# microsoft/esvit

Hardware: NVIDIA H100
Metric: multi-crop images/sec, Swin-T W7 pretrain step (2 global 224^2 + 8 local 96^2 crops, DDINOLoss V+R, K=65536) (higher is better)
Workload: dtype bf16

## Files before the change

esvit_b200/_lib.py:

```python
from __future__ import annotations

import ctypes
import os
from ctypes import c_double, c_float, c_int, c_longlong, c_void_p

HERE = os.path.dirname(os.path.abspath(__file__))
LIB_PATH = os.path.join(HERE, "lib", "libesvit_b200.so")
HEADER_PATH = os.path.join(os.path.dirname(HERE), "include", "esvit_b200.h")

ERR_BAD_ARG = 1001

P, I, L, F, D = c_void_p, c_int, c_longlong, c_float, c_double

SIGNATURES = {
    "esvit_add_ln_fwd": [P, P, P, I, P, P, F, P, P, I, P, P, L, I, P],
    "esvit_add_ln_bwd": [P, I, P, P, P, P, P, P, I, P, P, P, P, P, L, I, P],
    "esvit_patch_merge_ln_fwd": [P, P, P, F, P, P, P, I, I, I, I, P],
    "esvit_patch_merge_ln_bwd": [P, P, P, P, P, P, P, P, I, I, I, I, P],
    "esvit_token_mean_fwd": [P, P, I, I, I, P],
    "esvit_token_mean_bwd": [P, P, P, I, I, I, P],
    "esvit_patch_embed_fwd": [P, P, P, P, P, F, P, P, P, I, I, I, I, P],
    "esvit_patch_embed_bwd": [P, P, P, P, P, P, P, P, P, P, P, I, I, I, I, P],
    "esvit_window_attn_expand_bias": [P, P, I, I, P],
    "esvit_window_attn_fwd": [P, P, P, P, I, P, P, I, I, I, I, I, I, I, F, P],
    "esvit_window_attn_bwd": [P, P, P, P, I, P, P, P, P, P, P, I, I, I, I, I, I, I, F, P],
    "esvit_window_attn_probs": [P, P, P, P, I, P, I, I, I, I, I, I, I, F, P],
    "esvit_gemm_bias_act": [P, P, P, P, P, L, I, I, I, P],
    "esvit_gemm_mul_colsum": [P, P, P, P, P, P, L, I, I, P],
    "esvit_gemm_bf16": [P, P, P, P, P, L, I, I, I, I, I, I, P],
    "esvit_gemm_mul_colsum2": [P, P, P, P, P, P, L, I, I, I, I, P],
    "esvit_gemm_wgrad_ws_floats": [I, I],
    "esvit_gemm_wgrad": [P, P, P, P, L, I, I, I, I, P],
    "esvit_mlp_fwd": [P, P, P, P, P, P, P, P, L, I, P],
    "esvit_gelu_fwd": [P, P, L, P],
    "esvit_gelu_bwd": [P, P, P, L, P],
    "esvit_gelu_bwd_dbias": [P, P, P, P, L, I, P],
    "esvit_mul_bwd_dbias": [P, P, P, P, L, I, P],
    "esvit_l2norm_fwd": [P, P, P, F, L, I, P],
    "esvit_l2norm_bwd": [P, P, P, P, L, I, P],
    "esvit_weight_norm_fwd": [P, P, P, P, L, I, P],
    "esvit_weight_norm_bwd": [P, P, P, P, I, P, P, L, I, P],
    "esvit_row_lse": [P, P, F, P, L, I, P],
    "esvit_dino_ce_fwd": [P, P, P, P, P, P, P, F, F, P, L, I, P],
    "esvit_dino_ce_bwd": [P, P, P, P, P, P, P, P, P, F, F, P, L, I, P],
    "esvit_weighted_sum": [P, P, I, P, P],
    "esvit_row_softmax_q_max_k": [],
    "esvit_row_softmax_q": [P, P, F, P, P, L, I, P],
    "esvit_dino_ce_q_fwd": [P, P, P, P, P, F, P, L, I, P],
    "esvit_dino_ce_q_bwd": [P, P, P, P, P, P, P, F, P, L, I, P],
    "esvit_mixup_q_kpad": [I],
    "esvit_mixup_q": [P, P, I, I, I, F, P, P, P, P],
    "esvit_colsum_workspace_rows": [],
    "esvit_colsum": [P, L, I, P, P, P],
    "esvit_center_ema": [P, P, F, F, P, I, P],
    "esvit_normalize_rows": [P, P, L, I, F, P],
    "esvit_region_match": [P, P, I, I, I, I, I, P, P, P],
# ... 75 lines not shown
    if rc != 0:
        if rc == ERR_BAD_ARG:
            raise ValueError(f"{name}: unsupported shape / argument (ESVIT_ERR_BAD_ARG)")
        raise EsvitKernelError(f"{name} failed: {_cuda_error_string(rc)} (status {rc})")


_LAUNCHES = {"esvit_colsum": 2, "esvit_gemm_mul_colsum": 2, "esvit_gemm_mul_colsum2": 2, "esvit_gemm_wgrad": 2,
             "esvit_mixup_q": 2}
_launch_count = 0
_timed_names = set()
_timed_events = []
_META = {
    "esvit_dino_ce_bwd": lambda a: {"rows": int(a[-3]), "K": int(a[-2])},
    "esvit_window_attn_bwd": lambda a: _attn_meta(a),
    "esvit_window_attn_fwd": lambda a: _attn_meta(a),
    "esvit_window_attn_probs": lambda a: _attn_meta(a),
    "esvit_gemm_bias_act": lambda a: {"M": int(a[5]), "N": int(a[6]), "K": int(a[7])},
    "esvit_gemm_mul_colsum": lambda a: {"M": int(a[6]), "N": int(a[7]), "K": int(a[8])},
    "esvit_gemm_bf16": lambda a: {"M": int(a[5]), "N": int(a[6]), "K": int(a[7]), "b_mn": int(a[9]), "act": int(a[10]),
                                  "pre": a[4] is not None and a[4].value is not None},
    "esvit_gemm_mul_colsum2": lambda a: {"M": int(a[6]), "N": int(a[7]), "K": int(a[8])},
    "esvit_gemm_wgrad": lambda a: {"T": int(a[4]), "N": int(a[5]), "K": int(a[6])},
    "esvit_mlp_fwd": lambda a: {"M": int(a[8]), "C": int(a[9]), "student": a[6] is not None and a[6].value is not None},
    "esvit_add_ln_fwd": lambda a: {"T": int(a[-3]), "C": int(a[-2]), "has_x": a[0] is not None and a[0].value is not None,
                                   "has_delta": a[1] is not None and a[1].value is not None},
    "esvit_add_ln_bwd": lambda a: {"T": int(a[-3]), "C": int(a[-2])},
    "esvit_dino_ce_fwd": lambda a: {"rows": int(a[-3]), "K": int(a[-2])},
    "esvit_dino_ce_q_fwd": lambda a: {"rows": int(a[-3]), "K": int(a[-2])},
    "esvit_dino_ce_q_bwd": lambda a: {"rows": int(a[-3]), "K": int(a[-2])},
    "esvit_row_softmax_q": lambda a: {"rows": int(a[-3]), "K": int(a[-2])},
    "esvit_mixup_q": lambda a: {"ncrops": int(a[2]), "B": int(a[3]), "K": int(a[4])},
    "esvit_conv_im2col": lambda a: {"B": int(a[3]), "C": int(a[4]), "H": int(a[5]), "W": int(a[6]), "k": int(a[7]),
                                    "s": int(a[8]), "p": int(a[9]), "Kp": int(a[10])},
    "esvit_conv_col2im": lambda a: {"B": int(a[2]), "C": int(a[3]), "H": int(a[4]), "W": int(a[5]), "k": int(a[6]),
                                    "s": int(a[7]), "p": int(a[8]), "Kp": int(a[9])},
    "esvit_dwbn_fwd_stats": lambda a: {"B": int(a[5]), "H": int(a[6]), "W": int(a[7]), "Hp": int(a[8]), "Wp": int(a[9]),
                                       "C": int(a[10])},
    "esvit_dwbn_fwd_apply": lambda a: {"N": int(a[9]), "C": int(a[10])},
    "esvit_dwbn_bwd_stats": lambda a: {"N": int(a[7]), "C": int(a[8])},
    "esvit_dwbn_bwd_apply": lambda a: {"B": int(a[10]), "H": int(a[11]), "W": int(a[12]), "Hp": int(a[13]),
                                       "Wp": int(a[14]), "C": int(a[15])},
    "esvit_mhsa_win_fwd": lambda a: {"B": int(a[3]), "H": int(a[4]), "W": int(a[5]), "w": int(a[6]), "C": int(a[7]),
                                     "nH": int(a[8])},
    "esvit_mhsa_win_bwd": lambda a: {"B": int(a[6]), "H": int(a[7]), "W": int(a[8]), "w": int(a[9]), "C": int(a[10]),
                                     "nH": int(a[11])},
    "esvit_vil_sc_fwd": lambda a: {"B": int(a[8]), "nx": int(a[9]), "ny": int(a[10]), "nH": int(a[11])},
# ... 70 lines not shown
```

esvit_b200/backbone.py:

```python
from __future__ import annotations

from typing import Dict, List, Optional, Sequence

import torch
import torch.nn as nn

from . import ops, shadow

Tensor = torch.Tensor


class _CastCache:

    def __init__(self):
        self.d: Dict[int, Tensor] = {}

    def __call__(self, p: Optional[Tensor]) -> Optional[Tensor]:
        if p is None:
            return None
        k = id(p)
        t = self.d.get(k)
        if t is None:
            t = self.d[k] = shadow.as_bf16(p)
        return t
# ... 37 lines not shown
    r = torch.rand(kp.shape[0], samples, dtype=torch.float32, device=device)
    return r.add_(kp).floor_().div_(kp)


def row_samples(owner: nn.Module, counts, device) -> Tensor:
    counts = tuple(counts)

    def make():
        rows = torch.tensor([L for B, L in counts for _ in range(B)])
        return torch.arange(rows.numel()).repeat_interleave(rows).to(device)
    return _cached(owner, ("rows", counts, device), make)


def drop_path_rows(owner: nn.Module, scales: Optional[Tensor], counts, device) -> Optional[Tensor]:
    return None if scales is None else scales.index_select(1, row_samples(owner, counts, device))


def block_keeps(block: nn.Module, B: int, L: int, device) -> List[Optional[Tensor]]:
    ks = [drop_path_scales(block, [block.drop_prob], B, device) for _ in range(2)]
    return [None if k is None else drop_path_rows(block, k, ((B, L),), device)[0] for k in ks]


def pre_norm_block(x: Optional[Tensor], pend, norm1: nn.Module, attend, norm2: nn.Module, attn_bias: Optional[Tensor],
                   mlp, mlp_bias: Optional[Tensor], k1: Optional[Tensor], k2: Optional[Tensor]):
    delta, keep, dbias = pend if pend is not None else (None, None, None)
    x, y = ops.add_layer_norm(x, delta, keep, norm1.weight, norm1.bias, norm1.eps, delta_bias=dbias)
    x, y = ops.add_layer_norm(x, attend(y), k1, norm2.weight, norm2.bias, norm2.eps, delta_bias=attn_bias)
    return x, (mlp(y), k2, mlp_bias)


def tap(taps, b: int, x: Tensor, pend, geometry):
    if taps is None or taps[b] is None:
        return x, pend
    x = ops.residual_add(x, *pend)
    taps[b](x, geometry)
    return x, None


def check_crops(imgs: Sequence[Tensor]) -> None:
    for im in imgs:
        if im.dim() != 4 or im.shape[1] != 3:
            raise ValueError(f"expected crops [B, 3, H, W], got {tuple(im.shape)}")


class MultiCropBackbone(nn.Module):

    def _final_norm(self, x: Tensor, pend) -> Tensor:
        delta, keep, dbias = pend if pend is not None else (None, None, None)
        _, y = ops.add_layer_norm(x, delta, keep, self.norm.weight, self.norm.bias, self.norm.eps, y_bf16=False,
                                  delta_bias=dbias)
# ... 42 lines not shown
```

esvit_b200/csrc/gemm2_wgmma.cu:

```cuda
#include <cuda.h>

#include "common.cuh"

namespace hg {

constexpr int BK = 64;
constexpr int FOLD_THREADS = 64;
constexpr int SMEM_LIMIT = 232448;
enum { EPI_BIAS = 0, EPI_GELU = 1, EPI_MUL = 2, EPI_F32 = 3 };

__device__ __forceinline__ uint32_t smem_u32(const void* p) { return (uint32_t)__cvta_generic_to_shared(p); }
__device__ __forceinline__ void mbar_init(uint64_t* bar, uint32_t count) {
  asm volatile("mbarrier.init.shared::cta.b64 [%0], %1;\n" ::"r"(smem_u32(bar)), "r"(count));
}
__device__ __forceinline__ void mbar_expect_tx(uint64_t* bar, uint32_t bytes) {
  asm volatile("mbarrier.arrive.expect_tx.shared::cta.b64 _, [%0], %1;\n" ::"r"(smem_u32(bar)), "r"(bytes) : "memory");
}
__device__ __forceinline__ void mbar_arrive(uint64_t* bar) {
  asm volatile("mbarrier.arrive.shared::cta.b64 _, [%0];\n" ::"r"(smem_u32(bar)) : "memory");
}
__device__ __forceinline__ uint64_t global_ns() {
  uint64_t t;
  asm volatile("mov.u64 %0, %%globaltimer;\n" : "=l"(t));
  return t;
}
__device__ __forceinline__ void mbar_wait(uint64_t* bar, uint32_t parity) {
  const uint32_t a = smem_u32(bar);
  uint32_t done = 0;
  uint64_t t0 = 0;
  for (uint32_t it = 0;; ++it) {
    asm volatile(
        "{\n\t.reg .pred p;\n\t"
// ... 134 lines not shown
__device__ __forceinline__ float gelu_fwd(float x) {
  const float x2 = x * x;
  const float th = tanh_approx(x * fmaf(GELU_B, x2, GELU_A));
  const float hx = 0.5f * x;
  return fmaf(hx, th, hx);
}
__device__ __forceinline__ float gelu_fwd_grad(float x, float& dy) {
  const float x2 = x * x;
  const float th = tanh_approx(x * fmaf(GELU_B, x2, GELU_A));
  const float hx = 0.5f * x;
  const float m = fmaf(th, th, -1.f);
  const float nc = fmaf(-3.f * GELU_B, x2, -GELU_A);
  dy = fmaf(hx * m, nc, fmaf(0.5f, th, 0.5f));
  return fmaf(hx, th, hx);
}
constexpr float QGELU_A = 1.702f;
__device__ __forceinline__ float qgelu_fwd(float x) { return x * __frcp_rn(1.f + __expf(-QGELU_A * x)); }
__device__ __forceinline__ float qgelu_fwd_grad(float x, float& dy) {
  const float s = __frcp_rn(1.f + __expf(-QGELU_A * x));
  dy = s * fmaf(QGELU_A * x, 1.f - s, 1.f);
  return x * s;
}

struct Params {
  const float* bias;
  bf16* out;
  bf16* aux;
  float* colsum;
  float* part;
  int M, N, K;
  int splits;
  int kb_per_split;
};

template <int WG, int BN, int EPI>
struct Cfg {
  static constexpr bool PP = WG == 1;
  static constexpr int NEP = PP ? 2 : 1;
  static constexpr int BM = 64 * WG;
  static constexpr int A_BYTES = BM * BK * 2;
  static constexpr int B_BYTES = BN * BK * 2;
  static constexpr int STAGE_BYTES = A_BYTES + B_BYTES;
  static constexpr int BAR_BYTES = PP ? 512 : 256;
  static constexpr int NCHUNK = BN / 64;
  static constexpr int CHUNK_BYTES = BM * 128;
  static constexpr int EP_WG_BYTES = EPI == EPI_BIAS ? 2 * CHUNK_BYTES
                                   : EPI == EPI_GELU ? 4 * CHUNK_BYTES
                                   : EPI == EPI_MUL  ? NCHUNK * CHUNK_BYTES : 0;
  static constexpr int EP_BYTES = NEP * EP_WG_BYTES;
  static constexpr int CS_BYTES = EPI == EPI_MUL ? 8 * BN * 4 : 0;
  static constexpr int STAGES_RAW = (SMEM_LIMIT - 1024  - BAR_BYTES - EP_BYTES - CS_BYTES) / STAGE_BYTES;
  static constexpr int STAGES = STAGES_RAW > 6 ? 6 : STAGES_RAW;
  static constexpr int SMEM = 1024 + STAGES * STAGE_BYTES + EP_BYTES + CS_BYTES + BAR_BYTES;
  static constexpr int NTHREADS = 384;
  static_assert(STAGES >= (BN == 256 && (WG == 2 || EPI == EPI_MUL) ? 3 : 4), "operand ring too shallow");
  static_assert(SMEM <= SMEM_LIMIT, "shared memory budget");
  static_assert((2 * STAGES + 2 * NEP + 2 * NEP * NCHUNK + 2) * 8 <= BAR_BYTES, "mbarrier area");
};

template <int WG, int BN, int EPI, int AMN, int BMN, bool QUICK = false>
__global__ void __launch_bounds__(384, 1) gemm_kernel(const __grid_constant__ CUtensorMap map_a,
                                                      const __grid_constant__ CUtensorMap map_b,
                                                      const __grid_constant__ CUtensorMap map_o,
                                                      const __grid_constant__ CUtensorMap map_x,
                                                      const Params p) {
  using C = Cfg<WG, BN, EPI>;
  constexpr int STAGES = C::STAGES, BM = C::BM, NCHUNK = C::NCHUNK;
  constexpr bool PP = C::PP;
  extern __shared__ __align__(1024) uint8_t smem_raw[];
// ... 94 lines not shown
    const int frag_row = row0 + warp * 16 + (lane >> 2);
    const int frag_col = 2 * (lane & 3);
    const uint32_t rows_off = PP ? 0u : (uint32_t)wg * 8192u;
    const int e = PP ? wg : 0;
    uint8_t* const my_ep = ep + e * C::EP_WG_BYTES;
    constexpr uint32_t KSTEP_A = AMN ? (2048 >> 4) : (32 >> 4), KSTEP_B = BMN ? (2048 >> 4) : (32 >> 4);
    int stage = 0;
    uint32_t phase = 0;
    int local = 0;
    for (int item = blockIdx.x; item < num_items; item += gridDim.x, local++) {
      const int tile = item % tiles_mn, split = item / tiles_mn;
      const int m0 = (tile / n_tiles) * BM, n0 = (tile % n_tiles) * BN;
      const int kb0 = split * p.kb_per_split;
      int kb1 = kb0 + p.kb_per_split; kb1 = kb1 < k_blocks ? kb1 : k_blocks;
      if constexpr (PP) {
        if ((local & 1) != wg) {
          stage += kb1 - kb0;
          while (stage >= STAGES) { stage -= STAGES; phase ^= 1; }
          continue;
        }
        if (local > 0) mbar_wait(&turn[wg], ((local - 1) >> 1) & 1);
      }
      const int use = PP ? local >> 1 : local;
      float acc[BN / 2];
      int prev = -1;
      for (int kb = kb0; kb < kb1; kb++) {
        mbar_wait(&full[stage], phase);
        const uint32_t sa = smem_u32(tiles + stage * C::STAGE_BYTES) + rows_off;
        const uint64_t da = make_smem_desc(sa, AMN), db = make_smem_desc(smem_u32(tiles + stage * C::STAGE_BYTES) + C::A_BYTES, BMN);
        wgmma_fence();
#pragma unroll
        for (int k = 0; k < BK / 16; k++)
          wgmma_tile<BN, AMN, BMN>(acc, da + k * KSTEP_A, db + k * KSTEP_B, (kb > kb0 || k != 0) ? 1u : 0u);
        wgmma_commit();
        wgmma_wait<1>();
        if (prev >= 0) mbar_arrive(&empty[prev]);
        prev = stage;
        if (++stage == STAGES) { stage = 0; phase ^= 1; }
      }
      if constexpr (PP) mbar_arrive(&turn[wg ^ 1]);
      wgmma_wait<0>();
      if (prev >= 0) mbar_arrive(&empty[prev]);

      if constexpr (EPI == EPI_F32) {
#pragma unroll
        for (int i = 0; i < BN / 8; i++) {
          const int col = n0 + i * 8 + frag_col;
          if (col >= p.N) continue;
#pragma unroll
          for (int h = 0; h < 2; h++) {
            const int row = m0 + frag_row + 8 * h;
            if (row >= p.M) continue;
            const long long off = (long long)row * p.N + col;
            *reinterpret_cast<float2*>(p.part + (long long)split * p.M * p.N + off) =
                make_float2(acc[4 * i + 2 * h], acc[4 * i + 2 * h + 1]);
          }
        }
        continue;
      }

      if constexpr (EPI == EPI_MUL) mbar_wait(&cs_empty[e], (use & 1) ^ 1);
      const uint32_t lrow = (uint32_t)(warp * 16 + (lane & 15)) * 128u, lsw = lane & 7, lblk = lane >> 4;
      const bool leader = t == 0;
#pragma unroll
      for (int c = 0; c < NCHUNK; c++) {
        uint32_t buf;
        if constexpr (EPI == EPI_MUL) {
          buf = smem_u32(my_ep + c * C::CHUNK_BYTES) + rows_off;
          mbar_wait(&mul_full[e * NCHUNK + c], use & 1);
        } else {
          buf = smem_u32(my_ep + (c & 1) * (EPI == EPI_GELU ? 2 : 1) * C::CHUNK_BYTES) + rows_off;
        }
#pragma unroll
        for (int jj = 0; jj < 8; jj += 2) {
          const int i = c * 8 + jj;
          const uint32_t addr = buf + lrow + (((jj + lblk) ^ lsw) << 4);
          const float* a0 = acc + 4 * i;
          if constexpr (EPI == EPI_MUL) {
            uint32_t m[4];
            ldmatrix_x4(addr, m[0], m[1], m[2], m[3]);
            uint32_t o[4];
            float cs[2][2] = {{0.f, 0.f}, {0.f, 0.f}};
#pragma unroll
            for (int q = 0; q < 4; q++) {
              const float2 mf = unpack_bf162(m[q]);
              o[q] = pack_bf162(a0[2 * q] * mf.x, a0[2 * q + 1] * mf.y);
              const float2 of = unpack_bf162(o[q]);
              cs[q >> 1][0] += of.x; cs[q >> 1][1] += of.y;
            }
            stmatrix_x4(addr, o[0], o[1], o[2], o[3]);
#pragma unroll
            for (int s = 0; s < 2; s++) {
              float cs0 = cs[s][0], cs1 = cs[s][1];
#pragma unroll
              for (int o2 = 4; o2 < 32; o2 <<= 1) {
                cs0 += __shfl_xor_sync(0xffffffffu, cs0, o2);
                cs1 += __shfl_xor_sync(0xffffffffu, cs1, o2);
              }
              if (lane < 4)
                *reinterpret_cast<float2*>(cs_part + (wg * 4 + warp) * BN + (i + s) * 8 + frag_col) = make_float2(cs0, cs1);
            }
          } else {
            float b[4] = {0.f, 0.f, 0.f, 0.f};
            if (p.bias) {
#pragma unroll
              for (int s = 0; s < 2; s++) {
                const int col = n0 + (i + s) * 8 + frag_col;
                if (col < p.N) {
                  const float2 bb = __ldg(reinterpret_cast<const float2*>(p.bias + col));
                  b[2 * s] = bb.x; b[2 * s + 1] = bb.y;
                }
              }
            }
            uint32_t o[4], d[4];
#pragma unroll
            for (int q = 0; q < 4; q++) {
              const float v0 = a0[2 * q] + b[2 * (q >> 1)], v1 = a0[2 * q + 1] + b[2 * (q >> 1) + 1];
              if constexpr (EPI == EPI_GELU) {
                if (p.aux) {
                  float d0, d1;
                  float y0, y1;
                  if constexpr (QUICK) {
                    y0 = qgelu_fwd_grad(v0, d0); y1 = qgelu_fwd_grad(v1, d1);
                  } else {
// ... 385 lines not shown
    if (!c.a_mn) return c.b_mn ? launch_cfg<WG, BN, EPI, 0, 1>(c, stream, rows_out) : launch_cfg<WG, BN, EPI, 0, 0>(c, stream, rows_out);
    return c.b_mn ? launch_cfg<WG, BN, EPI, 1, 1>(c, stream, rows_out) : launch_cfg<WG, BN, EPI, 1, 0>(c, stream, rows_out);
  }
  return ESVIT_ERR_BAD_ARG;
}

template <int EPI>
static int launch_epi(const Call& c, int wg, int bn, void* stream, int* rows_out) {
  if (wg == 2 && bn == 256) return launch_majors<2, 256, EPI>(c, stream, rows_out);
  if (wg == 2 && bn == 128) return launch_majors<2, 128, EPI>(c, stream, rows_out);
  if (wg == 1 && bn == 256) return launch_majors<1, 256, EPI>(c, stream, rows_out);
  if (wg == 1 && bn == 128) return launch_majors<1, 128, EPI>(c, stream, rows_out);
  return ESVIT_ERR_BAD_ARG;
}

static int launch_quick(const Call& c, int wg, int bn, void* stream) {
  if (c.a_mn || c.b_mn) return ESVIT_ERR_BAD_ARG;
  if (wg == 2 && bn == 256) return launch_cfg<2, 256, EPI_GELU, 0, 0, true>(c, stream, nullptr);
  if (wg == 2 && bn == 128) return launch_cfg<2, 128, EPI_GELU, 0, 0, true>(c, stream, nullptr);
  if (wg == 1 && bn == 256) return launch_cfg<1, 256, EPI_GELU, 0, 0, true>(c, stream, nullptr);
  if (wg == 1 && bn == 128) return launch_cfg<1, 128, EPI_GELU, 0, 0, true>(c, stream, nullptr);
  return ESVIT_ERR_BAD_ARG;
}

static int launch(const Call& c, int epi, int wg, int bn, void* stream, int* rows_out = nullptr) {
  switch (epi) {
    case EPI_BIAS: return launch_epi<EPI_BIAS>(c, wg, bn, stream, rows_out);
    case EPI_GELU: return launch_epi<EPI_GELU>(c, wg, bn, stream, rows_out);
    case EPI_MUL: return launch_epi<EPI_MUL>(c, wg, bn, stream, rows_out);
    case EPI_F32: return launch_epi<EPI_F32>(c, wg, bn, stream, rows_out);
  }
  return ESVIT_ERR_BAD_ARG;
}

static bool pads_more(long long n, int wide, int narrow) {
  return (n + wide - 1) / wide * wide > (n + narrow - 1) / narrow * narrow;
}
static void pick_tile(long long M, int N, int K, int tile, bool fit_n, int* wg, int* bn) {
  tile %= 10000;
  if (tile > 0) { *wg = tile / 1000; *bn = tile % 1000; return; }
  const int sms = esvit_num_sms();
  const bool narrow = fit_n && (pads_more(N, 256, 128) || K <= 256);
  const int cand[4][2] = {{2, 256}, {2, 128}, {1, 256}, {1, 128}};
  for (const auto& cd : cand) {
    if (cd[1] == 256 && (N <= 128 || narrow)) continue;
    const long long items = ((M + 64 * cd[0] - 1) / (64 * cd[0])) * ((N + cd[1] - 1) / cd[1]);
// ... 74 lines not shown
  c.p.M = N; c.p.N = K; c.p.K = (int)T; c.p.splits = splits; c.p.kb_per_split = kbs;
  const int rc = hg::launch(c, hg::EPI_F32, wg, bn, stream);
  if (rc != 0) return rc;
  const long long n4 = (long long)N * K / 4;
  hg::split_fold_kernel<<<(unsigned)((n4 + 255) / 256), 256, 0, (cudaStream_t)stream>>>(ws, splits, n4, dw, accumulate);
  ESVIT_LAUNCH_CHECK();
}

ESVIT_API int esvit_mlp_fwd(const void* x, const void* w1, const float* b1, const void* w2, const float* b2, void* y,
                            void* h, void* gelu_grad, long long M, int C, void* stream) {
  auto aligned = [](const void* q, uintptr_t a) { return ((uintptr_t)q & (a - 1)) == 0; };
  if (M <= 0 || M > 0x7fffffffLL || !x || !w1 || !w2 || !y || (h == nullptr) != (gelu_grad == nullptr)) return ESVIT_ERR_BAD_ARG;
  if (!aligned(x, 16) || !aligned(w1, 16) || !aligned(w2, 16) || !aligned(y, 16) || !aligned(h, 16) ||
      !aligned(gelu_grad, 16) || !aligned(b1, 8) || !aligned(b2, 8))
    return ESVIT_ERR_BAD_ARG;
  switch (C) {
    case 96: return hg::mlp_launch_c<96>(x, w1, b1, w2, b2, y, h, gelu_grad, (int)M, stream);
    case 128: return hg::mlp_launch_c<128>(x, w1, b1, w2, b2, y, h, gelu_grad, (int)M, stream);
    case 192: return hg::mlp_launch_c<192>(x, w1, b1, w2, b2, y, h, gelu_grad, (int)M, stream);
  }
  return ESVIT_ERR_BAD_ARG;
}

ESVIT_API int esvit_gemm_bias_act(const void* a, const void* w, const float* bias, void* out, void* pre, long long M,
                                  int N, int K, int act, void* stream) {
  return esvit_gemm_bf16(a, w, bias, out, pre, M, N, K, 0, 0, act, 0, stream);
}
ESVIT_API int esvit_gemm_mul_colsum(const void* a, const void* w, const void* mult, void* out, float* colsum, float* ws,
                                    long long M, int N, int K, void* stream) {
  return esvit_gemm_mul_colsum2(a, w, mult, out, colsum, ws, M, N, K, 0, 0, stream);
}
```

esvit_b200/linear.py:

```python
from __future__ import annotations

from typing import Optional

import torch
from torch.autograd import Function
from torch.autograd.function import once_differentiable

from . import ops

Tensor = torch.Tensor
BF16 = torch.bfloat16
F32 = torch.float32


def _wgrad(key, dy2: Tensor, x2: Tensor, shape):
    d = ops._Arena.accs
    if d is None:
        return ops.gemm_wgrad(dy2, x2).view(shape)
    buf = d.get(key)
    if buf is not None and tuple(buf.shape) == tuple(shape):
        ops.gemm_wgrad(dy2, x2, out=buf, accumulate=True)
        return None
    buf = d[key] = ops.gemm_wgrad(dy2, x2).view(shape)
    return buf.view(shape)


class LinearFn(Function):

    @staticmethod
    def forward(ctx, x, wp, w16, bias):
        y = ops.gemm(x, w16, bias)
        ctx.save_for_backward(x, w16)
        ctx.wkey = ("w", wp.data_ptr())
        ctx.wshape = tuple(wp.shape)
        return y

    @staticmethod
    @once_differentiable
    def backward(ctx, g):
        x, w16 = ctx.saved_tensors
        g = ops._chk(g, BF16, "g")
        N, K = w16.shape
        g2 = g.reshape(-1, N)
        dx = ops.gemm(g2, w16, None, b_mn=True).view(x.shape) if ctx.needs_input_grad[0] else None
        dw = _wgrad(ctx.wkey, g2, x.reshape(-1, K), ctx.wshape) if ctx.needs_input_grad[1] else None
        return dx, dw, None, None


class MlpFn(Function):

    @staticmethod
    def forward(ctx, x, w1p, w1, b1, w2p, w2, b2, act: int = 1):
        need = any(ctx.needs_input_grad)
        C = x.shape[-1]
        if act == 1 and C in ops.MLP_FUSED_C and w1.shape[0] == 4 * C:
            if need:
                y, h, pre = ops.mlp_fwd(x, w1, b1, w2, b2, want_h=True)
            else:
                y, h, pre = ops.mlp_fwd(x, w1, b1, w2, b2), None, None
        else:
            if need:
                h, pre = ops.gemm(x, w1, b1, act=act, want_pre=True)
            else:
                h, pre = ops.gemm(x, w1, b1, act=act), None
            y = ops.gemm(h, w2, b2)
        ctx.save_for_backward(x, w1, w2, pre, h)
        ctx.keys = (("w", w1p.data_ptr()), tuple(w1p.shape), ("w", w2p.data_ptr()), tuple(w2p.shape))
        ctx.bias_meta = (b1.shape, b1.device, b1.data_ptr())
        return y
# ... 72 lines not shown
```

esvit_b200/ops.py:

```python
from __future__ import annotations

import ctypes
from typing import List, Optional, Sequence, Tuple

import torch
from torch.autograd import Function
from torch.autograd.function import once_differentiable

from . import _lib, shadow

Tensor = torch.Tensor
BF16 = torch.bfloat16
F32 = torch.float32


def _p(t: Optional[Tensor]):
    return ctypes.c_void_p(t.data_ptr()) if t is not None else None


def _po(t: Tensor, off_elems: int):
    return ctypes.c_void_p(t.data_ptr() + off_elems * t.element_size())


def _stream():
# ... 72 lines not shown
    return (xout if delta is not None else x), y, mean, rstd


class AddLayerNormFn(Function):

    @staticmethod
    def forward(ctx, x, delta, dbias, keep, gamma, beta, eps: float, y_bf16: bool):
        x = _chk(x, F32, "x")
        delta = _chk(delta, BF16, "delta")
        dbias = _chk(dbias, F32, "delta_bias")
        keep = _chk(keep, F32, "keep")
        gamma, beta = _chk(gamma, F32, "gamma"), _chk(beta, F32, "beta")
        ref = x if x is not None else delta
        tps = ref.numel() // ref.shape[-1] // ref.shape[0]
        xout, y, mean, rstd = _add_ln_fwd(x, delta, keep, tps, gamma, beta, eps, True, y_bf16)
        ctx.save_for_backward(xout, mean, rstd, gamma, keep)
        ctx.tps, ctx.y_bf16, ctx.has_dbias, ctx.has_x = tps, y_bf16, dbias is not None, x is not None
        return xout, y

    @staticmethod
    @once_differentiable
    def backward(ctx, g_xout, g_y):
        xout, mean, rstd, gamma, keep = ctx.saved_tensors
        T, C = xout.numel() // xout.shape[-1], xout.shape[-1]
        g_xout = _chk(g_xout, F32, "g_xout") if g_xout is not None else None
        if g_y is not None:
            g_y = _chk(g_y, BF16 if ctx.y_bf16 else F32, "g_y")
        dx = torch.empty_like(xout) if ctx.has_x else None
        ddelta = torch.empty(xout.shape, dtype=BF16, device=xout.device)
        acc, first = _acc(("add_ln", gamma.data_ptr()), (3, C), xout.device)
        _lib.call("esvit_add_ln_bwd", _p(g_y), 1 if ctx.y_bf16 else 0, _p(g_xout), _p(xout), _p(mean), _p(rstd),
                  _p(gamma), _p(keep), ctx.tps, _p(dx), _p(ddelta), _p(acc[0]), _p(acc[1]),
                  _p(acc[2]) if ctx.has_dbias else None, T, C, _stream())
        if not first:
            return dx, ddelta, None, None, None, None, None, None
        return dx, ddelta, (acc[2] if ctx.has_dbias else None), None, acc[0], acc[1], None, None


class LayerNormFn(Function):

    @staticmethod
    def forward(ctx, x, gamma, beta, eps: float, y_bf16: bool):
        x = _chk(x, F32, "x")
        gamma, beta = _chk(gamma, F32, "gamma"), _chk(beta, F32, "beta")
        _, y, mean, rstd = _add_ln_fwd(x, None, None, 1, gamma, beta, eps, True, y_bf16)
        ctx.save_for_backward(x, mean, rstd, gamma)
        ctx.y_bf16 = y_bf16
        return y

    @staticmethod
    @once_differentiable
    def backward(ctx, g_y):
        x, mean, rstd, gamma = ctx.saved_tensors
        T, C = x.numel() // x.shape[-1], x.shape[-1]
        g_y = _chk(g_y, BF16 if ctx.y_bf16 else F32, "g_y")
        dx = torch.empty_like(x)
        acc, first = _acc(("ln", gamma.data_ptr()), (2, C), x.device)
        _lib.call("esvit_add_ln_bwd", _p(g_y), 1 if ctx.y_bf16 else 0, None, _p(x), _p(mean), _p(rstd), _p(gamma),
                  None, 1, _p(dx), None, _p(acc[0]), _p(acc[1]), None, T, C, _stream())
# ... 486 lines not shown
    M = a.numel() // K
    N = b.shape[1] if b_mn else b.shape[0]
    out = torch.empty_like(mult)
    ws = torch.empty(GEMM_COLSUM_WS_ROWS * N, dtype=F32, device=a.device)
    _lib.call("esvit_gemm_mul_colsum2", _p(a), _p(b), _p(mult), _p(out), _p(colsum), _p(ws), M, N, K, 1 if b_mn else 0, tile,
              _stream())
    return out


MLP_FUSED_C = (96, 128, 192)


def mlp_fwd(x: Tensor, w1: Tensor, b1: Optional[Tensor], w2: Tensor, b2: Optional[Tensor], want_h: bool = False):
    x, w1, w2 = _chk(x, BF16, "x"), _chk(w1, BF16, "w1"), _chk(w2, BF16, "w2")
    b1, b2 = _chk(b1, F32, "b1"), _chk(b2, F32, "b2")
    C = x.shape[-1]
    M = x.numel() // C
    assert tuple(w1.shape) == (4 * C, C) and tuple(w2.shape) == (C, 4 * C), (x.shape, w1.shape, w2.shape)
    y = torch.empty_like(x)
    h = torch.empty(*x.shape[:-1], 4 * C, dtype=BF16, device=x.device) if want_h else None
    pre = torch.empty_like(h) if want_h else None
    _lib.call("esvit_mlp_fwd", _p(x), _p(w1), _p(b1), _p(w2), _p(b2), _p(y), _p(h), _p(pre), M, C, _stream())
    return (y, h, pre) if want_h else y


_wgrad_ws = {}


def gemm_wgrad(dy: Tensor, x: Tensor, out: Optional[Tensor] = None, accumulate: bool = False, tile: int = 0) -> Tensor:
    dy, x = _chk(dy, BF16, "dy"), _chk(x, BF16, "x")
    N, K = dy.shape[-1], x.shape[-1]
    T = dy.numel() // N
    assert x.numel() // K == T
    if out is None:
        out = torch.empty(N, K, dtype=F32, device=dy.device)
        accumulate = False
    key = (dy.device, N, K)
    ws = _wgrad_ws.get(key)
    if ws is None:
        n = _lib.load().esvit_gemm_wgrad_ws_floats(N, K)
        if n <= 0:
            raise ValueError("esvit_gemm_wgrad: weight too large for the split-K workspace")
        ws = _wgrad_ws[key] = torch.empty(n, dtype=F32, device=dy.device)
    _lib.call("esvit_gemm_wgrad", _p(dy), _p(x), _p(out), _p(ws), T, N, K, 1 if accumulate else 0, tile, _stream())
    return out

# ... 739 lines not shown
```

esvit_b200/swin_transformer.py:

```python
from __future__ import annotations

import math
import os
from functools import partial
from typing import List, Optional, Sequence

import torch
import torch.nn as nn
import torch.nn.functional as F

from . import backbone, linear, ops, shadow
from .backbone import MultiCropBackbone, _CastCache

Tensor = torch.Tensor
BF16 = torch.bfloat16


USE_TCGEN05_FC1 = os.environ.get("ESVIT_TCGEN05_FC1", "1") != "0"
USE_GEMM2 = os.environ.get("ESVIT_GEMM2", "1") != "0"


def _trunc_normal_(t: Tensor, std: float = .02) -> Tensor:
    return nn.init.trunc_normal_(t, std=std)

# ... 56 lines not shown
    def __init__(self, dim, window_size, num_heads, qkv_bias=True, qk_scale=None, attn_drop=0., proj_drop=0.):
        super().__init__()
        self.dim = dim
        self.window_size = tuple(window_size)
        self.num_heads = num_heads
        head_dim = dim // num_heads
        self.scale = qk_scale or head_dim ** -0.5
        if head_dim != 32 or self.window_size[0] != self.window_size[1] or attn_drop != 0. or proj_drop != 0.:
            raise NotImplementedError("kernel supports head_dim 32, square windows, no attention dropout")
        if not qkv_bias:
            raise NotImplementedError("qkv_bias=False is not used by any EsViT config")
        ws = self.window_size[0]
        self.relative_position_bias_table = nn.Parameter(torch.zeros((2 * ws - 1) * (2 * ws - 1), num_heads))
        t = torch.arange(ws * ws)
        y, x = t // ws, t % ws
        idx = (y[:, None] - y[None, :] + ws - 1) * (2 * ws - 1) + (x[:, None] - x[None, :] + ws - 1)
        self.register_buffer("relative_position_index", idx)
        self.qkv = nn.Linear(dim, dim * 3, bias=True)
        self.proj = nn.Linear(dim, dim)
        _trunc_normal_(self.relative_position_bias_table, std=.02)

    def attend(self, y: Tensor, grp, shift: int, cc: Optional[_CastCache] = None,
               maps: Optional[List[Tensor]] = None) -> Tensor:
        qkv = _lin_c(y, self.qkv, cc)
        ws = self.window_size[0]
        bexp = None if cc is None else cc.expanded_bias(self.relative_position_bias_table, self.num_heads, ws)
        a = ops.WindowAttentionGroupsFn.apply(qkv, self.qkv.bias, self.relative_position_bias_table, tuple(grp),
                                              self.num_heads, ws, shift, float(self.scale), bexp)
        if maps is not None:
            (B, H, W, _), = grp
            maps.append(ops.window_attention_probs(qkv.view(B, H * W, -1), self.qkv.bias,
                                                   self.relative_position_bias_table, H, W, self.num_heads, ws, shift,
                                                   float(self.scale), bexp))
        return _lin_c(a, self.proj, cc)

    def forward(self, x: Tensor, mask: Optional[Tensor] = None):
        if mask is not None:
            raise NotImplementedError("explicit masks are generated in-kernel; call SwinTransformerBlock instead")
        ws = self.window_size[0]
        B_, N, C = x.shape
        assert N == ws * ws
        return self.attend(x.to(BF16).reshape(B_ * N, C), ((B_, ws, ws, 0),), 0).view(B_, N, C), None


class SwinTransformerBlock(nn.Module):
    def __init__(self, dim, input_resolution, num_heads, window_size=7, shift_size=0, mlp_ratio=4., qkv_bias=True,
                 qk_scale=None, drop=0., attn_drop=0., drop_path=0., act_layer=nn.GELU, norm_layer=nn.LayerNorm):
        super().__init__()
        self.dim, self.input_resolution, self.num_heads = dim, input_resolution, num_heads
        self.window_size, self.shift_size, self.mlp_ratio = window_size, shift_size, mlp_ratio
        if min(self.input_resolution) <= self.window_size:
            self.shift_size = 0
            self.window_size = min(self.input_resolution)
        assert 0 <= self.shift_size < self.window_size
        self.norm1 = norm_layer(dim)
        self.attn = WindowAttention(dim, (self.window_size, self.window_size), num_heads, qkv_bias, qk_scale,
                                    attn_drop, drop)
        self.drop_prob = float(drop_path)
        self.norm2 = norm_layer(dim)
        self.mlp = Mlp(dim, int(dim * mlp_ratio), act_layer=act_layer, drop=drop)

    def fused(self, x: Optional[Tensor], pending, grp, cc: Optional[_CastCache], k1: Optional[Tensor],
              k2: Optional[Tensor], maps: Optional[List[Tensor]] = None):
        return backbone.pre_norm_block(x, pending, self.norm1,
                                       lambda y: self.attn.attend(y, grp, self.shift_size, cc, maps), self.norm2,
                                       self.attn.proj.bias, lambda y: self.mlp.fused(y, cc), self.mlp.fc2.bias, k1, k2)

    def forward(self, x: Tensor):
        xs, grp = _one_group(x.float())
        xs, pend = self.fused(xs, None, grp, None, *backbone.block_keeps(self, x.shape[0], x.shape[1], x.device))
        return ops.residual_add(xs, *pend).view(x.shape), None


class PatchMerging(nn.Module):
    def __init__(self, input_resolution, dim, norm_layer=nn.LayerNorm):
        super().__init__()
        self.input_resolution, self.dim = input_resolution, dim
        self.reduction = nn.Linear(4 * dim, 2 * dim, bias=False)
        self.norm = norm_layer(4 * dim)

    def forward(self, x: Tensor) -> Tensor:
        xs, grp = _one_group(x)
        m, _ = self.fused(xs, grp)
        return m.float().view(x.shape[0], -1, m.shape[-1])

    def fused(self, x: Tensor, grp, cc: Optional[_CastCache] = None):
        y = ops.PatchMergeLNGroupsFn.apply(x, self.norm.weight, self.norm.bias, self.norm.eps, tuple(grp))
        new_grp, row0 = [], 0
        for B, H, W, _ in grp:
# ... 212 lines not shown
```

include/esvit_b200.h:

```cpp
#ifndef ESVIT_B200_H
#define ESVIT_B200_H

#ifdef __cplusplus
extern "C" {
#endif

#define ESVIT_ERR_BAD_ARG 1001

int esvit_add_ln_fwd(const float* x, const void* delta, const float* keep, int tokens_per_sample,
                     const float* gamma, const float* beta, float eps, float* xout, void* y, int y_is_bf16,
                     float* mean, float* rstd, long long T, int C, void* stream);
int esvit_add_ln_bwd(const void* dy, int dy_is_bf16, const float* dxo, const float* xs, const float* mean,
                     const float* rstd, const float* gamma, const float* keep, int tokens_per_sample, float* dx,
                     void* ddelta, float* dgamma, float* dbeta, float* ddelta_bias, long long T, int C, void* stream);

int esvit_patch_merge_ln_fwd(const float* x, const float* gamma, const float* beta, float eps, void* y, float* mean,
                             float* rstd, int B, int H, int W, int C, void* stream);
int esvit_patch_merge_ln_bwd(const void* dy, const float* x, const float* mean, const float* rstd,
                             const float* gamma, float* dx, float* dgamma, float* dbeta, int B, int H, int W, int C,
                             void* stream);

int esvit_token_mean_fwd(const float* region, float* pooled, int B, int N, int C, void* stream);
int esvit_token_mean_bwd(const float* dpooled, const float* dregion_in, float* dregion, int B, int N, int C,
                         void* stream);
// ... 9 lines not shown
                          void* out, float* lse, int B, int H, int W, int C, int nH, int ws, int shift, float scale,
                          void* stream);
int esvit_window_attn_bwd(const void* qkv, const void* qkv_bias, const float* bias_table, float* bias_ws, int bias_ready,
                          const void* out, const void* dout, const float* lse, void* dqkv, float* dbias_table,
                          float* dqkv_bias, int B, int H, int W, int C, int nH, int ws, int shift, float scale,
                          void* stream);
int esvit_window_attn_probs(const void* qkv, const void* qkv_bias, const float* bias_table, float* bias_ws, int bias_ready,
                            float* probs, int B, int H, int W, int C, int nH, int ws, int shift, float scale, void* stream);

int esvit_gemm_bias_act(const void* a, const void* w, const float* bias, void* out, void* pre, long long M, int N, int K,
                        int act, void* stream);
int esvit_gemm_mul_colsum(const void* a, const void* w, const void* mult, void* out, float* colsum, float* ws,
                          long long M, int N, int K, void* stream);

int esvit_gemm_bf16(const void* a, const void* b, const float* bias, void* out, void* pre, long long M, int N, int K,
                    int a_mn, int b_mn, int act, int tile, void* stream);
int esvit_gemm_mul_colsum2(const void* a, const void* b, const void* mult, void* out, float* colsum, float* ws,
                           long long M, int N, int K, int b_mn, int tile, void* stream);
int esvit_gemm_wgrad_ws_floats(int N, int K);
int esvit_gemm_wgrad(const void* dy, const void* x, float* dw, float* ws, long long T, int N, int K, int accumulate,
                     int tile, void* stream);
int esvit_mlp_fwd(const void* x, const void* w1, const float* b1, const void* w2, const float* b2, void* y, void* h,
                  void* gelu_grad, long long M, int C, void* stream);

int esvit_gelu_fwd(const void* x, void* y, long long n, void* stream);
int esvit_gelu_bwd(const void* x, const void* dy, void* dx, long long n, void* stream);
int esvit_gelu_bwd_dbias(const void* x, const void* dy, void* dx, float* dbias, long long R, int N, void* stream);
int esvit_mul_bwd_dbias(const void* gp, const void* dy, void* dx, float* dbias, long long R, int N, void* stream);

int esvit_l2norm_fwd(const void* x, void* y, float* inv, float eps, long long R, int D, void* stream);
int esvit_l2norm_bwd(const void* x, const void* dy, const float* inv, void* dx, long long R, int D, void* stream);
int esvit_weight_norm_fwd(const float* v, const float* g, void* w, float* norm, long long K, int D, void* stream);
int esvit_weight_norm_bwd(const float* v, const float* g, const float* norm, const void* dw, int dw_is_f32, float* dv,
                          float* dg, long long K, int D, void* stream);

int esvit_row_lse(const void* x, const float* center, float inv_temp, float* lse, long long R, int K, void* stream);
int esvit_dino_ce_fwd(const void* s, const void* t, const float* center, float* lse_s, const float* lse_t,
                      const int* trow, const int* order, float inv_temp_t, float inv_tau_s, float* row_loss, long long R,
                      int K, void* stream);
int esvit_dino_ce_bwd(const void* s, const void* t, const float* center, const float* lse_s, const float* lse_t,
                      const int* trow, const int* order, const float* w, const float* gscale, float inv_temp_t,
                      float inv_tau_s, void* ds, long long R, int K, void* stream);
int esvit_weighted_sum(const float* v, const float* w, int R, float* out, void* stream);
int esvit_row_softmax_q_max_k(void);
int esvit_row_softmax_q(const void* x, const float* center, float inv_temp, float* lse, void* q, long long R, int K,
                        void* stream);
// ... 104 lines not shown
```

Before: 1366.

## Fuse attention output projection GEMM with residual add and LayerNorm epilogue

Adds a WGMMA GEMM epilogue (EPI_LN) that adds bias, applies drop-path keep scaling, adds the fp32 residual, computes the row LayerNorm statistics and writes both the new residual and the bf16 normalized output. Swin blocks with dim at most 128 (stage 1) now use it for the attention proj + norm2 step. This removes the separate proj output tensor and the standalone add_ln kernel pass. The cost is that one full-row N=128 tile is forced per CTA and the epilogue does extra global loads and register pressure. Backward is reorganized to reuse the existing add_ln backward and linear backward.

Result: no change. 1373 (median of 6 runs) (+0.6%).

```diff
diff --git a/esvit_b200/_lib.py b/esvit_b200/_lib.py
--- a/esvit_b200/_lib.py
+++ b/esvit_b200/_lib.py
@@ -32,6 +32,7 @@
     "esvit_gemm_wgrad_ws_floats": [I, I],
     "esvit_gemm_wgrad": [P, P, P, P, L, I, I, I, I, P],
     "esvit_mlp_fwd": [P, P, P, P, P, P, P, P, L, I, P],
+    "esvit_gemm_add_ln": [P, P, P, P, P, P, P, F, P, P, P, P, L, I, I, P],
     "esvit_gelu_fwd": [P, P, L, P],
     "esvit_gelu_bwd": [P, P, P, L, P],
     "esvit_gelu_bwd_dbias": [P, P, P, P, L, I, P],
@@ -153,6 +154,7 @@
     "esvit_gemm_mul_colsum2": lambda a: {"M": int(a[6]), "N": int(a[7]), "K": int(a[8])},
     "esvit_gemm_wgrad": lambda a: {"T": int(a[4]), "N": int(a[5]), "K": int(a[6])},
     "esvit_mlp_fwd": lambda a: {"M": int(a[8]), "C": int(a[9]), "student": a[6] is not None and a[6].value is not None},
+    "esvit_gemm_add_ln": lambda a: {"M": int(a[12]), "N": int(a[13]), "K": int(a[14])},
     "esvit_add_ln_fwd": lambda a: {"T": int(a[-3]), "C": int(a[-2]), "has_x": a[0] is not None and a[0].value is not None,
                                    "has_delta": a[1] is not None and a[1].value is not None},
     "esvit_add_ln_bwd": lambda a: {"T": int(a[-3]), "C": int(a[-2])},
diff --git a/esvit_b200/backbone.py b/esvit_b200/backbone.py
--- a/esvit_b200/backbone.py
+++ b/esvit_b200/backbone.py
@@ -83,10 +83,13 @@
 
 
 def pre_norm_block(x: Optional[Tensor], pend, norm1: nn.Module, attend, norm2: nn.Module, attn_bias: Optional[Tensor],
-                   mlp, mlp_bias: Optional[Tensor], k1: Optional[Tensor], k2: Optional[Tensor]):
+                   mlp, mlp_bias: Optional[Tensor], k1: Optional[Tensor], k2: Optional[Tensor], attend_ln=None):
     delta, keep, dbias = pend if pend is not None else (None, None, None)
     x, y = ops.add_layer_norm(x, delta, keep, norm1.weight, norm1.bias, norm1.eps, delta_bias=dbias)
-    x, y = ops.add_layer_norm(x, attend(y), k1, norm2.weight, norm2.bias, norm2.eps, delta_bias=attn_bias)
+    if attend_ln is not None:
+        x, y = attend_ln(x, y, k1)
+    else:
+        x, y = ops.add_layer_norm(x, attend(y), k1, norm2.weight, norm2.bias, norm2.eps, delta_bias=attn_bias)
     return x, (mlp(y), k2, mlp_bias)
 
 
diff --git a/esvit_b200/csrc/gemm2_wgmma.cu b/esvit_b200/csrc/gemm2_wgmma.cu
--- a/esvit_b200/csrc/gemm2_wgmma.cu
+++ b/esvit_b200/csrc/gemm2_wgmma.cu
@@ -7,7 +7,7 @@
 constexpr int BK = 64;
 constexpr int FOLD_THREADS = 64;
 constexpr int SMEM_LIMIT = 232448;
-enum { EPI_BIAS = 0, EPI_GELU = 1, EPI_MUL = 2, EPI_F32 = 3 };
+enum { EPI_BIAS = 0, EPI_GELU = 1, EPI_MUL = 2, EPI_F32 = 3, EPI_LN = 4 };
 
 __device__ __forceinline__ uint32_t smem_u32(const void* p) { return (uint32_t)__cvta_generic_to_shared(p); }
 __device__ __forceinline__ void mbar_init(uint64_t* bar, uint32_t count) {
@@ -188,6 +188,101 @@
   return x * s;
 }
 
+struct LnParams {
+  const float* x;
+  const float* keep;
+  const float* gamma;
+  const float* beta;
+  float* xout;
+  float* mean;
+  float* rstd;
+  float eps;
+};
+
+__device__ __forceinline__ void prefetch_rows_l2(const float* x, int row0, int M, int n, int t) {
+  const int rows = M - row0 < 64 ? M - row0 : 64;
+  if (rows <= 0) return;
+  const char* base = reinterpret_cast<const char*>(x + (long long)row0 * n);
+  for (int o = t * 128; o < rows * n * 4; o += 128 * 128) asm volatile("prefetch.global.L2 [%0];\n" ::"l"(base + o));
+}
+
+template <int NB>
+__device__ __forceinline__ void res_ln_rows(float* acc, const float* bias, const LnParams& q, int row, int M,
+                                            int n, int c0, float (&mu)[2], float (&rs)[2]) {
+  const float inv_n = 1.f / (float)n;
+  float ks[2], s[2] = {0.f, 0.f};
+#pragma unroll
+  for (int h = 0; h < 2; h++) ks[h] = (q.keep && row + 8 * h < M) ? __ldg(q.keep + row + 8 * h) : 1.f;
+  constexpr int CH = 4;
+#pragma unroll
+  for (int i0 = 0; i0 < NB; i0 += CH) {
+    float2 xv[CH][2];
+#pragma unroll
+    for (int i = i0; i < i0 + CH && i < NB; i++)
+#pragma unroll
+      for (int h = 0; h < 2; h++) {
+        const int r = row + 8 * h, col = 8 * i + c0;
+        xv[i - i0][h] = make_float2(0.f, 0.f);
+        if (col < n && r < M) xv[i - i0][h] = *reinterpret_cast<const float2*>(q.x + (long long)r * n + col);
+      }
+#pragma unroll
+    for (int i = i0; i < i0 + CH && i < NB; i++) {
+      const int col = 8 * i + c0;
+      if (col >= n) {
+        acc[4 * i] = acc[4 * i + 1] = acc[4 * i + 2] = acc[4 * i + 3] = 0.f;
+        continue;
+      }
+      float2 b = make_float2(0.f, 0.f);
+      if (bias) b = *reinterpret_cast<const float2*>(bias + col);
+#pragma unroll
+      for (int h = 0; h < 2; h++) {
+        const int r = row + 8 * h;
+        float* a = acc + 4 * i + 2 * h;
+        const float2 d = unpack_bf162(pack_bf162(a[0] + b.x, a[1] + b.y));
+        a[0] = fmaf(ks[h], d.x, xv[i - i0][h].x);
+        a[1] = fmaf(ks[h], d.y, xv[i - i0][h].y);
+        if (r < M) *reinterpret_cast<float2*>(q.xout + (long long)r * n + col) = make_float2(a[0], a[1]);
+        s[h] += a[0] + a[1];
+      }
+    }
+  }
+  float v[2] = {0.f, 0.f};
+#pragma unroll
+  for (int h = 0; h < 2; h++) {
+    s[h] += __shfl_xor_sync(0xffffffffu, s[h], 1);
+    s[h] += __shfl_xor_sync(0xffffffffu, s[h], 2);
+    mu[h] = s[h] * inv_n;
+  }
+#pragma unroll
+  for (int i = 0; i < NB; i++) {
+    if (8 * i + c0 >= n) continue;
+#pragma unroll
+    for (int h = 0; h < 2; h++) {
+      const float a = acc[4 * i + 2 * h] - mu[h], b = acc[4 * i + 2 * h + 1] - mu[h];
+      acc[4 * i + 2 * h] = a; acc[4 * i + 2 * h + 1] = b;
+      v[h] += a * a + b * b;
+    }
+  }
+#pragma unroll
+  for (int h = 0; h < 2; h++) {
+    v[h] += __shfl_xor_sync(0xffffffffu, v[h], 1);
+    v[h] += __shfl_xor_sync(0xffffffffu, v[h], 2);
+    rs[h] = rsqrtf(v[h] * inv_n + q.eps);
+    const int r = row + 8 * h;
+    if (c0 == 0 && r < M) { q.mean[r] = mu[h]; q.rstd[r] = rs[h]; }
+  }
+}
+__device__ __forceinline__ uint32_t ln_pack(const float* a, float rs, float2 g, float2 b) {
+  return pack_bf162(a[0] * rs * g.x + b.x, a[1] * rs * g.y + b.y);
+}
+__device__ __forceinline__ void ln_affine(const LnParams& q, int col, int n, float2& g, float2& b) {
+  g = b = make_float2(0.f, 0.f);
+  if (col < n) {
+    g = *reinterpret_cast<const float2*>(q.gamma + col);
+    b = *reinterpret_cast<const float2*>(q.beta + col);
+  }
+}
+
 struct Params {
   const float* bias;
   bf16* out;
@@ -197,6 +292,7 @@
   int M, N, K;
   int splits;
   int kb_per_split;
+  LnParams ln;
 };
 
 template <int WG, int BN, int EPI>
@@ -210,7 +306,7 @@
   static constexpr int BAR_BYTES = PP ? 512 : 256;
   static constexpr int NCHUNK = BN / 64;
   static constexpr int CHUNK_BYTES = BM * 128;
-  static constexpr int EP_WG_BYTES = EPI == EPI_BIAS ? 2 * CHUNK_BYTES
+  static constexpr int EP_WG_BYTES = EPI == EPI_BIAS || EPI == EPI_LN ? 2 * CHUNK_BYTES
                                    : EPI == EPI_GELU ? 4 * CHUNK_BYTES
                                    : EPI == EPI_MUL  ? NCHUNK * CHUNK_BYTES : 0;
   static constexpr int EP_BYTES = NEP * EP_WG_BYTES;
@@ -351,6 +447,7 @@
         if (local > 0) mbar_wait(&turn[wg], ((local - 1) >> 1) & 1);
       }
       const int use = PP ? local >> 1 : local;
+      if constexpr (EPI == EPI_LN) prefetch_rows_l2(p.ln.x, m0 + row0, p.M, p.N, t);
       float acc[BN / 2];
       int prev = -1;
       for (int kb = kb0; kb < kb1; kb++) {
@@ -389,6 +486,8 @@
       }
 
       if constexpr (EPI == EPI_MUL) mbar_wait(&cs_empty[e], (use & 1) ^ 1);
+      float mu[2] = {0.f, 0.f}, rs[2] = {0.f, 0.f};
+      if constexpr (EPI == EPI_LN) res_ln_rows<BN / 8>(acc, p.bias, p.ln, m0 + frag_row, p.M, p.N, frag_col, mu, rs);
       const uint32_t lrow = (uint32_t)(warp * 16 + (lane & 15)) * 128u, lsw = lane & 7, lblk = lane >> 4;
       const bool leader = t == 0;
 #pragma unroll
@@ -429,6 +528,14 @@
               if (lane < 4)
                 *reinterpret_cast<float2*>(cs_part + (wg * 4 + warp) * BN + (i + s) * 8 + frag_col) = make_float2(cs0, cs1);
             }
+          } else if constexpr (EPI == EPI_LN) {
+            float2 g[2], be[2];
+#pragma unroll
+            for (int s = 0; s < 2; s++) ln_affine(p.ln, (i + s) * 8 + frag_col, p.N, g[s], be[s]);
+            uint32_t o[4];
+#pragma unroll
+            for (int q = 0; q < 4; q++) o[q] = ln_pack(a0 + 2 * q, rs[q & 1], g[q >> 1], be[q >> 1]);
+            stmatrix_x4(addr, o[0], o[1], o[2], o[3]);
           } else {
             float b[4] = {0.f, 0.f, 0.f, 0.f};
             if (p.bias) {
@@ -860,6 +967,7 @@
   if (wg == 1 && bn == 128) return launch_cfg<1, 128, EPI_GELU, 0, 0, true>(c, stream, nullptr);
   return ESVIT_ERR_BAD_ARG;
 }
+
 
 static int launch(const Call& c, int epi, int wg, int bn, void* stream, int* rows_out = nullptr) {
   switch (epi) {
@@ -980,6 +1088,33 @@
   return ESVIT_ERR_BAD_ARG;
 }
 
+static bool ln_args(const float* x, const float* gamma, const float* beta, const float* xout, const void* y,
+                    const float* mean, const float* rstd, const float* bias) {
+  auto aligned = [](const void* q, uintptr_t a) { return ((uintptr_t)q & (a - 1)) == 0; };
+  return x && gamma && beta && xout && y && mean && rstd && aligned(x, 8) && aligned(xout, 8) && aligned(gamma, 8) &&
+         aligned(beta, 8) && aligned(bias, 8) && aligned(y, 16);
+}
+static hg::LnParams ln_params(const float* x, const float* keep, const float* gamma, const float* beta, float eps,
+                              float* xout, float* mean, float* rstd) {
+  hg::LnParams q;
+  q.x = x; q.keep = keep; q.gamma = gamma; q.beta = beta; q.xout = xout; q.mean = mean; q.rstd = rstd; q.eps = eps;
+  return q;
+}
+
+ESVIT_API int esvit_gemm_add_ln(const void* a, const void* w, const float* bias, const float* x, const float* keep,
+                                const float* gamma, const float* beta, float eps, float* xout, void* y, float* mean,
+                                float* rstd, long long M, int N, int K, void* stream) {
+  if (M <= 0 || N <= 0 || K <= 0 || N > 128 || (N % 8) || (K % 8) || M > 0x7fffffffLL ||
+      !ln_args(x, gamma, beta, xout, y, mean, rstd, bias))
+    return ESVIT_ERR_BAD_ARG;
+  hg::Call c;
+  c.a = a; c.b = w; c.a_mn = 0; c.b_mn = 0;
+  c.p.bias = bias; c.p.out = (bf16*)y; c.p.aux = nullptr; c.p.colsum = nullptr; c.p.part = nullptr;
+  c.p.M = (int)M; c.p.N = N; c.p.K = K; c.p.splits = 1; c.p.kb_per_split = (K + hg::BK - 1) / hg::BK;
+  c.p.ln = ln_params(x, keep, gamma, beta, eps, xout, mean, rstd);
+  return hg::launch_cfg<2, 128, hg::EPI_LN, 0, 0>(c, stream, nullptr);
+}
+
 ESVIT_API int esvit_gemm_bias_act(const void* a, const void* w, const float* bias, void* out, void* pre, long long M,
                                   int N, int K, int act, void* stream) {
   return esvit_gemm_bf16(a, w, bias, out, pre, M, N, K, 0, 0, act, 0, stream);
diff --git a/esvit_b200/linear.py b/esvit_b200/linear.py
--- a/esvit_b200/linear.py
+++ b/esvit_b200/linear.py
@@ -39,12 +39,36 @@
     @once_differentiable
     def backward(ctx, g):
         x, w16 = ctx.saved_tensors
-        g = ops._chk(g, BF16, "g")
-        N, K = w16.shape
-        g2 = g.reshape(-1, N)
-        dx = ops.gemm(g2, w16, None, b_mn=True).view(x.shape) if ctx.needs_input_grad[0] else None
-        dw = _wgrad(ctx.wkey, g2, x.reshape(-1, K), ctx.wshape) if ctx.needs_input_grad[1] else None
+        dx, dw = _linear_backward(g, x, w16, ctx.wkey, ctx.wshape, *ctx.needs_input_grad[:2])
         return dx, dw, None, None
+
+
+def _linear_backward(g, x, w16, wkey, wshape, need_x: bool, need_w: bool):
+    g = ops._chk(g, BF16, "g")
+    N, K = w16.shape
+    g2 = g.reshape(-1, N)
+    dx = ops.gemm(g2, w16, None, b_mn=True).view(x.shape) if need_x else None
+    dw = _wgrad(wkey, g2, x.reshape(-1, K), wshape) if need_w else None
+    return dx, dw
+
+
+class LinearAddLNFn(Function):
+
+    @staticmethod
+    def forward(ctx, x, a, wp, w16, bias, keep, gamma, beta, eps: float):
+        xout, y, mean, rstd = ops.gemm_add_ln(a, w16, bias, x, keep, gamma, beta, eps)
+        ctx.save_for_backward(xout, mean, rstd, gamma, keep, a, w16)
+        ctx.wkey, ctx.wshape, ctx.has_bias = ("w", wp.data_ptr()), tuple(wp.shape), bias is not None
+        return xout, y
+
+    @staticmethod
+    @once_differentiable
+    def backward(ctx, g_xout, g_y):
+        xout, mean, rstd, gamma, keep, a, w16 = ctx.saved_tensors
+        dx, ddelta, db, dgamma, dbeta = ops.add_ln_backward(g_xout, g_y, xout, mean, rstd, gamma, keep, 1, True, True,
+                                                            ctx.has_bias)
+        da, dw = _linear_backward(ddelta, a, w16, ctx.wkey, ctx.wshape, *ctx.needs_input_grad[1:3])
+        return dx, da, dw, None, db, None, dgamma, dbeta, None
 
 
 class MlpFn(Function):
diff --git a/esvit_b200/ops.py b/esvit_b200/ops.py
--- a/esvit_b200/ops.py
+++ b/esvit_b200/ops.py
@@ -118,19 +118,25 @@
     @once_differentiable
     def backward(ctx, g_xout, g_y):
         xout, mean, rstd, gamma, keep = ctx.saved_tensors
-        T, C = xout.numel() // xout.shape[-1], xout.shape[-1]
-        g_xout = _chk(g_xout, F32, "g_xout") if g_xout is not None else None
-        if g_y is not None:
-            g_y = _chk(g_y, BF16 if ctx.y_bf16 else F32, "g_y")
-        dx = torch.empty_like(xout) if ctx.has_x else None
-        ddelta = torch.empty(xout.shape, dtype=BF16, device=xout.device)
-        acc, first = _acc(("add_ln", gamma.data_ptr()), (3, C), xout.device)
-        _lib.call("esvit_add_ln_bwd", _p(g_y), 1 if ctx.y_bf16 else 0, _p(g_xout), _p(xout), _p(mean), _p(rstd),
-                  _p(gamma), _p(keep), ctx.tps, _p(dx), _p(ddelta), _p(acc[0]), _p(acc[1]),
-                  _p(acc[2]) if ctx.has_dbias else None, T, C, _stream())
-        if not first:
-            return dx, ddelta, None, None, None, None, None, None
-        return dx, ddelta, (acc[2] if ctx.has_dbias else None), None, acc[0], acc[1], None, None
+        dx, ddelta, ddb, dgamma, dbeta = add_ln_backward(g_xout, g_y, xout, mean, rstd, gamma, keep, ctx.tps, ctx.y_bf16,
+                                                         ctx.has_x, ctx.has_dbias)
+        return dx, ddelta, ddb, None, dgamma, dbeta, None, None
+
+
+def add_ln_backward(g_xout, g_y, xout, mean, rstd, gamma, keep, tps: int, y_bf16: bool, has_x: bool, has_dbias: bool):
+    T, C = xout.numel() // xout.shape[-1], xout.shape[-1]
+    g_xout = _chk(g_xout, F32, "g_xout") if g_xout is not None else None
+    if g_y is not None:
+        g_y = _chk(g_y, BF16 if y_bf16 else F32, "g_y")
+    dx = torch.empty_like(xout) if has_x else None
+    ddelta = torch.empty(xout.shape, dtype=BF16, device=xout.device)
+    acc, first = _acc(("add_ln", gamma.data_ptr()), (3, C), xout.device)
+    _lib.call("esvit_add_ln_bwd", _p(g_y), 1 if y_bf16 else 0, _p(g_xout), _p(xout), _p(mean), _p(rstd),
+              _p(gamma), _p(keep), tps, _p(dx), _p(ddelta), _p(acc[0]), _p(acc[1]),
+              _p(acc[2]) if has_dbias else None, T, C, _stream())
+    if not first:
+        return dx, ddelta, None, None, None
+    return dx, ddelta, (acc[2] if has_dbias else None), acc[0], acc[1]
 
 
 class LayerNormFn(Function):
@@ -663,6 +669,29 @@
     pre = torch.empty_like(h) if want_h else None
     _lib.call("esvit_mlp_fwd", _p(x), _p(w1), _p(b1), _p(w2), _p(b2), _p(y), _p(h), _p(pre), M, C, _stream())
     return (y, h, pre) if want_h else y
+
+
+PROJ_LN_MAX_N = 128
+
+
+def _ln_outputs(x: Tensor):
+    T = x.numel() // x.shape[-1]
+    return (torch.empty_like(x), torch.empty(x.shape, dtype=BF16, device=x.device),
+            torch.empty(T, dtype=F32, device=x.device), torch.empty(T, dtype=F32, device=x.device))
+
+
+def gemm_add_ln(a: Tensor, w: Tensor, bias: Optional[Tensor], x: Tensor, keep: Optional[Tensor], gamma: Tensor,
+                beta: Tensor, eps: float):
+    a, w = _chk(a, BF16, "a"), _chk(w, BF16, "w")
+    bias, x, keep = _chk(bias, F32, "bias"), _chk(x, F32, "x"), _chk(keep, F32, "keep")
+    gamma, beta = _chk(gamma, F32, "gamma"), _chk(beta, F32, "beta")
+    N, K = w.shape
+    M = a.numel() // K
+    assert a.shape[-1] == K and x.shape[-1] == N and x.numel() == M * N, (a.shape, w.shape, x.shape)
+    xout, y, mean, rstd = _ln_outputs(x)
+    _lib.call("esvit_gemm_add_ln", _p(a), _p(w), _p(bias), _p(x), _p(keep), _p(gamma), _p(beta), eps, _p(xout), _p(y),
+              _p(mean), _p(rstd), M, N, K, _stream())
+    return xout, y, mean, rstd
 
 
 _wgrad_ws = {}
diff --git a/esvit_b200/swin_transformer.py b/esvit_b200/swin_transformer.py
--- a/esvit_b200/swin_transformer.py
+++ b/esvit_b200/swin_transformer.py
@@ -102,6 +102,16 @@
 
     def attend(self, y: Tensor, grp, shift: int, cc: Optional[_CastCache] = None,
                maps: Optional[List[Tensor]] = None) -> Tensor:
+        return _lin_c(self._attention(y, grp, shift, cc, maps), self.proj, cc)
+
+    def attend_ln(self, x: Tensor, y: Tensor, keep: Optional[Tensor], norm: nn.Module, grp, shift: int,
+                  cc: Optional[_CastCache] = None, maps: Optional[List[Tensor]] = None):
+        a = self._attention(y, grp, shift, cc, maps)
+        w16 = shadow.as_bf16(self.proj.weight, track_grad=False) if cc is None else cc.nograd(self.proj.weight)
+        return linear.LinearAddLNFn.apply(x, a, self.proj.weight, w16, self.proj.bias, keep, norm.weight, norm.bias,
+                                          norm.eps)
+
+    def _attention(self, y: Tensor, grp, shift: int, cc: Optional[_CastCache], maps: Optional[List[Tensor]]) -> Tensor:
         qkv = _lin_c(y, self.qkv, cc)
         ws = self.window_size[0]
         bexp = None if cc is None else cc.expanded_bias(self.relative_position_bias_table, self.num_heads, ws)
@@ -112,7 +122,7 @@
             maps.append(ops.window_attention_probs(qkv.view(B, H * W, -1), self.qkv.bias,
                                                    self.relative_position_bias_table, H, W, self.num_heads, ws, shift,
                                                    float(self.scale), bexp))
-        return _lin_c(a, self.proj, cc)
+        return a
 
     def forward(self, x: Tensor, mask: Optional[Tensor] = None):
         if mask is not None:
@@ -142,9 +152,13 @@
 
     def fused(self, x: Optional[Tensor], pending, grp, cc: Optional[_CastCache], k1: Optional[Tensor],
               k2: Optional[Tensor], maps: Optional[List[Tensor]] = None):
+        attend_ln = None
+        if USE_GEMM2 and self.dim <= ops.PROJ_LN_MAX_N:
+            attend_ln = lambda x, y, k: self.attn.attend_ln(x, y, k, self.norm2, grp, self.shift_size, cc, maps)
         return backbone.pre_norm_block(x, pending, self.norm1,
                                        lambda y: self.attn.attend(y, grp, self.shift_size, cc, maps), self.norm2,
-                                       self.attn.proj.bias, lambda y: self.mlp.fused(y, cc), self.mlp.fc2.bias, k1, k2)
+                                       self.attn.proj.bias, lambda y: self.mlp.fused(y, cc), self.mlp.fc2.bias, k1, k2,
+                                       attend_ln)
 
     def forward(self, x: Tensor):
         xs, grp = _one_group(x.float())
diff --git a/include/esvit_b200.h b/include/esvit_b200.h
--- a/include/esvit_b200.h
+++ b/include/esvit_b200.h
@@ -55,6 +55,9 @@
                      int tile, void* stream);
 int esvit_mlp_fwd(const void* x, const void* w1, const float* b1, const void* w2, const float* b2, void* y, void* h,
                   void* gelu_grad, long long M, int C, void* stream);
+int esvit_gemm_add_ln(const void* a, const void* w, const float* bias, const float* x, const float* keep,
+                      const float* gamma, const float* beta, float eps, float* xout, void* y, float* mean, float* rstd,
+                      long long M, int N, int K, void* stream);
 
 int esvit_gelu_fwd(const void* x, void* y, long long n, void* stream);
 int esvit_gelu_bwd(const void* x, const void* dy, void* dx, long long n, void* stream);
```
